# graphcore-research/bess-kge

Hardware: AMD Instinct MI355X
Metric: positive+negative triples scored/sec (higher is better)
Workload: dtype f32; 1 GPU; ogbl-biokg-shaped ComplEx d=256 fp32 (W=512), 93,773 entities per shard, n_shard=1, S=4096 positives x 256 per-triple negatives per GPU per step, EmbeddingMoving, mode=score (gather+score+loss); negatives_per_triple=256, mode=score, collectives=none

## Files before the change

bess-kge_amd/csrc/neg_pertriple.hip:

```cpp
#include "common.h"
#include "loss_rows.h"

namespace bess {

struct NegPtArgs {
    const float* query;
    const void* base;
    const int32_t* idx;
    int64_t n_query;
    int n_neg;
    int W;
    int nch;
    int nb;
    int items_per_query;
    float sign;
    int accum = 0;
    float p = 2.f;
    int dn_by_row = 0;
    int sweep_shift = -1;
};

struct FuseArgs {
    const float* pos;
    int kind;
    float beta;
    float margin;
    float shift;
    float* st_ml;
    float* st_acc;
    const uint8_t* mask = nullptr;
    int64_t mask_rows = 0;
    int mask_cols = 0, mask_from = 0;
};

__device__ __forceinline__ float sigmoid_f(float x) { return 1.f / (1.f + expf(-x)); }

template <typename T, int VEC, int IT, int RED, int UNROLL, bool FUSE>
__global__ __launch_bounds__(256) void k_neg_pertriple_fwd(NegPtArgs a, float* __restrict__ out,
                                                           int64_t ld_out, FuseArgs f) {
    const int lane = threadIdx.x & 63;
    const int g = lane & 15;
    const int sub = lane >> 4;
    const int64_t item = blockIdx.x * 4ll + (threadIdx.x >> 6);
    if (item >= a.n_query * a.items_per_query) return;
    const int64_t q = item / a.items_per_query;
    const int k0 = static_cast<int>(item - q * a.items_per_query) * a.nb;
    const int k1 = min(k0 + a.nb, a.n_neg);

    float qv[IT][VEC];
    const float* qp = a.query + q * a.W;
#pragma unroll
    for (int it = 0; it < IT; ++it) {
        load_chunk<float, VEC>(qp, g + 16 * it, a.nch, qv[it]);
    }

    const T* base = static_cast<const T*>(a.base);
    const int32_t* idx = a.idx + q * a.n_neg;
    float* orow = out + q * ld_out;
    float fm = -INFINITY, fl = 0.f, facc[IT][VEC];
    float fpos = 0.f;
    if (FUSE) {
#pragma unroll
        for (int it = 0; it < IT; ++it)
#pragma unroll
            for (int v = 0; v < VEC; ++v) facc[it][v] = 0.f;
        if (f.kind == BESS_LOSS_MARGIN) fpos = f.pos[q];
    }

    int32_t nrow[UNROLL];
#pragma unroll
    for (int u = 0; u < UNROLL; ++u) nrow[u] = idx[min(k0 + sub + 4 * u, k1 - 1)];
    for (int kb = k0; kb < k1; kb += 4 * UNROLL) {
        float ev[UNROLL][IT][VEC];
        bool valid[UNROLL];
#pragma unroll
        for (int u = 0; u < UNROLL; ++u) {
            const int k = kb + sub + 4 * u;
            valid[u] = k < k1;
            const T* rp = base + static_cast<int64_t>(nrow[u]) * a.W;
            nrow[u] = idx[min(k + 4 * UNROLL, k1 - 1)];
#pragma unroll
            for (int it = 0; it < IT; ++it) {
                load_chunk<T, VEC>(rp, g + 16 * it, a.nch, ev[u][it]);
            }
        }
#pragma unroll
        for (int u = 0; u < UNROLL; ++u) {
            float acc = 0.f;
#pragma unroll
            for (int it = 0; it < IT; ++it) {
#pragma unroll
                for (int v = 0; v < VEC; ++v) {
                    if (RED == RED_DOT) {
                        acc = fmaf(qv[it][v], ev[u][it][v], acc);
                    } else if (RED == RED_L1) {
                        acc += fabsf(qv[it][v] - ev[u][it][v]);
                    } else {
                        acc += lp_term(qv[it][v] - ev[u][it][v], a.p);
                    }
                }
            }
            acc = row16_allreduce_sum(acc);
            if (RED == RED_L2) acc = lp_root(acc, a.p);
            float sc = a.sign * acc;
            if (FUSE && f.mask && valid[u]) {
                const int kcol = kb + sub + 4 * u - f.mask_from;
                const int64_t mrow = f.mask_rows == 1 ? 0 : q;
                if (kcol >= 0 && f.mask[mrow * f.mask_cols + kcol] == 0) sc += BESS_BAD_NEGATIVE_SCORE;
            }
            if (g == 0 && valid[u]) orow[kb + sub + 4 * u] = a.accum ? orow[kb + sub + 4 * u] + sc : sc;
            if (FUSE && valid[u]) {
                const float z = f.beta * (sc + f.shift);
                const float m_new = fmaxf(fm, z);
                const float corr = expf(fm - m_new);
                const float e = expf(z - m_new);
                float gs = 1.f;
                if (f.kind == BESS_LOSS_LOGSIGMOID) gs = sigmoid_f(sc + f.margin);
                else if (f.kind == BESS_LOSS_MARGIN) gs = (sc - fpos + f.margin > 0.f) ? 1.f : 0.f;
                const float p = e * gs;
                fl = fmaf(fl, corr, e);
                fm = m_new;
                const float inv_norm = RED == RED_L2 ? lp_inv(acc, a.p) : 0.f;
#pragma unroll
                for (int it = 0; it < IT; ++it)
#pragma unroll
                    for (int v = 0; v < VEC; ++v) {
                        float dsdq;
                        if (RED == RED_DOT) dsdq = ev[u][it][v];
                        else if (RED == RED_L1) dsdq = -sgnf(qv[it][v] - ev[u][it][v]);
                        else dsdq = -lp_dterm(qv[it][v] - ev[u][it][v], a.p) * inv_norm;
                        facc[it][v] = fmaf(facc[it][v], corr, p * dsdq);
                    }
            }
        }
    }
    if (FUSE) {
        float m_all = fmaxf(fm, __shfl_xor(fm, 16, 64));
        m_all = fmaxf(m_all, __shfl_xor(m_all, 32, 64));
        const float sc = (fm == -INFINITY) ? 0.f : expf(fm - m_all);
        float l = fl * sc;
        l += __shfl_xor(l, 16, 64);
        l += __shfl_xor(l, 32, 64);
        const int64_t slot = q * a.items_per_query + (item - q * a.items_per_query);
        if (lane == 0) {
            f.st_ml[slot * 2 + 0] = m_all;
            f.st_ml[slot * 2 + 1] = l;
        }
        float* ap = f.st_acc + slot * a.W;
#pragma unroll
        for (int it = 0; it < IT; ++it) {
            const int c = g + 16 * it;
#pragma unroll
            for (int v = 0; v < VEC; ++v) {
                float x = facc[it][v] * sc;
                x += __shfl_xor(x, 16, 64);
                x += __shfl_xor(x, 32, 64);
                if (sub == 0 && c < a.nch) ap[c * VEC + v] = x;
            }
        }
    }
}

constexpr int SW_NB = 1024;
constexpr int SW_PMAX = 8192;
constexpr int SW_PPT = SW_PMAX / 256;
constexpr int SW_SHARE = SW_PMAX / 8;
constexpr int SW_QFLOATS = 16384;
constexpr int64_t SW_REUSE_MIN = 4;

struct SweepArgs {
    int qb;
    int kc;
    int n_kchunks;
    int shift;
    int qstride;
};

template <typename T, int VEC, int IT, int RED, int UNROLL>
__global__ __launch_bounds__(256) void k_neg_pertriple_fwd_sweep(NegPtArgs a, SweepArgs s, float* __restrict__ out,
                                                                 int64_t ld_out) {
    extern __shared__ __attribute__((aligned(16))) float qs[];
    __shared__ int hist[SW_NB + 4];
    __shared__ int2 ent[SW_SHARE];
    __shared__ int rk[2][SW_PPT * 4];
    __shared__ int wsum[4];
    __shared__ int cut[4];

    const int tid = threadIdx.x;
    const int lane = tid & 63;
    const int wave = tid >> 6;
    const int label = blockIdx.x & 7;
    const int bc = blockIdx.x >> 3;
    const int qblk = bc / s.n_kchunks;
    const int kch = bc - qblk * s.n_kchunks;
    const int64_t q0 = static_cast<int64_t>(qblk) * s.qb;
    const int nqb = static_cast<int>(min(static_cast<int64_t>(s.qb), a.n_query - q0));
    const int kc0 = kch * s.kc;
    const int kcn = min(s.kc, a.n_neg - kc0);
    const int P = nqb * kcn;
    const int lo = static_cast<int>((static_cast<int64_t>(label) * P) >> 3);
    const int hi = static_cast<int>((static_cast<int64_t>(label + 1) * P) >> 3);

    for (int i = tid; i < nqb * IT * 16; i += 256) {
        const int qi = i / (IT * 16);
        const int c = i - qi * (IT * 16);
        float v[VEC];
        load_chunk<float, VEC>(a.query + (q0 + qi) * a.W, c, a.nch, v);
#pragma unroll
        for (int j = 0; j < VEC; ++j) qs[qi * s.qstride + c * VEC + j] = v[j];
    }
    for (int b = tid; b < SW_NB; b += 256) hist[b] = 0;
    if (tid < 2) cut[tid] = -1;
    int rr[SW_PPT];
#pragma unroll
    for (int j = 0; j < SW_PPT; ++j) {
        const int p = tid + 256 * j;
        rr[j] = 0;
        if (p < P) {
            const int qi = p / kcn;
            rr[j] = a.idx[(q0 + qi) * a.n_neg + kc0 + (p - qi * kcn)];
        }
    }
    __syncthreads();
#pragma unroll
    for (int j = 0; j < SW_PPT; ++j)
        if (tid + 256 * j < P) atomicAdd(&hist[min(static_cast<unsigned>(rr[j]) >> s.shift, SW_NB - 1u)], 1);
    __syncthreads();

    {
        int c[4], sum = 0;
#pragma unroll
        for (int i = 0; i < 4; ++i) {
            c[i] = hist[4 * tid + i];
            sum += c[i];
        }
        int incl = sum;
#pragma unroll
        for (int off = 1; off < 64; off <<= 1) {
            const int y = __shfl_up(incl, off, 64);
            if (lane >= off) incl += y;
        }
        if (lane == 63) wsum[wave] = incl;
        __syncthreads();
        int run = incl - sum;
        for (int w = 0; w < wave; ++w) run += wsum[w];
#pragma unroll
        for (int i = 0; i < 4; ++i) {
            const int b = 4 * tid + i;
            hist[b] = run;
            if (run < lo && lo < run + c[i]) cut[0] = b;
            if (run < hi && hi < run + c[i]) cut[1] = b;
            run += c[i];
        }
        if (tid == 255) hist[SW_NB] = run;
    }
    __syncthreads();

    const int cut0 = cut[0], cut1 = cut[1];
    const uint64_t lt = (1ull << lane) - 1ull;
#pragma unroll
    for (int j = 0; j < SW_PPT; ++j) {
        const bool live = tid + 256 * j < P;
        const unsigned b = min(static_cast<unsigned>(rr[j]) >> s.shift, SW_NB - 1u);
        const uint64_t m0 = __ballot(live && static_cast<int>(b) == cut0);
        const uint64_t m1 = __ballot(live && static_cast<int>(b) == cut1);
        if (lane == 0) {
            rk[0][j * 4 + wave] = __popcll(m0);
            rk[1][j * 4 + wave] = __popcll(m1);
        }
    }
    __syncthreads();
    if (wave == 0) {
#pragma unroll
        for (int h = 0; h < 2; ++h) {
            const int x0 = rk[h][2 * lane], x1 = rk[h][2 * lane + 1];
            int incl = x0 + x1;
#pragma unroll
            for (int off = 1; off < 64; off <<= 1) {
                const int y = __shfl_up(incl, off, 64);
                if (lane >= off) incl += y;
            }
            rk[h][2 * lane] = incl - x0 - x1;
            rk[h][2 * lane + 1] = incl - x1;
        }
    }
    __syncthreads();

    int slot[SW_PPT];
#pragma unroll
    for (int j = 0; j < SW_PPT; ++j) {
        const bool live = tid + 256 * j < P;
        const unsigned b = min(static_cast<unsigned>(rr[j]) >> s.shift, SW_NB - 1u);
        const bool in0 = live && static_cast<int>(b) == cut0;
        const bool in1 = live && static_cast<int>(b) == cut1 && !in0;
        const uint64_t m0 = __ballot(in0);
        const uint64_t m1 = __ballot(in1);
        const int b0 = live ? hist[b] : 0, b1 = live ? hist[b + 1] : 0;
        slot[j] = -1;
        if (live) {
            if (in0 || in1) {
                const int r = in0 ? rk[0][j * 4 + wave] + __popcll(m0 & lt) : rk[1][j * 4 + wave] + __popcll(m1 & lt);
                const int pos = b0 + r;
                if (pos >= lo && pos < hi) slot[j] = pos - lo;
            } else if (b0 >= lo && b1 <= hi) {
                slot[j] = -2;
            }
        }
    }
    __syncthreads();
#pragma unroll
    for (int j = 0; j < SW_PPT; ++j) {
        const int p = tid + 256 * j;
        if (slot[j] == -1) continue;
        const unsigned b = min(static_cast<unsigned>(rr[j]) >> s.shift, SW_NB - 1u);
        const int e = slot[j] >= 0 ? slot[j] : atomicAdd(&hist[b], 1) - lo;
        const int qi = p / kcn;
        ent[e] = make_int2(rr[j], (qi << 16) | (p - qi * kcn));
    }
    __syncthreads();

    const int n = hi - lo;
    const int g = lane & 15;
    const int sub = lane >> 4;
    const T* base = static_cast<const T*>(a.base);
    int2 nx[UNROLL];
#pragma unroll
    for (int u = 0; u < UNROLL; ++u) nx[u] = ent[max(0, min(wave * 4 * UNROLL + sub + 4 * u, n - 1))];
    for (int e0 = wave * 4 * UNROLL; e0 < n; e0 += 16 * UNROLL) {
        float ev[UNROLL][IT][VEC];
        int2 cur[UNROLL];
        bool valid[UNROLL];
#pragma unroll
        for (int u = 0; u < UNROLL; ++u) {
            const int e = e0 + sub + 4 * u;
            valid[u] = e < n;
            cur[u] = nx[u];
            const T* rp = base + static_cast<int64_t>(cur[u].x) * a.W;
            nx[u] = ent[min(e + 16 * UNROLL, n - 1)];
#pragma unroll
            for (int it = 0; it < IT; ++it) load_chunk<T, VEC>(rp, g + 16 * it, a.nch, ev[u][it]);
        }
#pragma unroll
        for (int u = 0; u < UNROLL; ++u) {
            const int qi = cur[u].y >> 16;
            const int kk = cur[u].y & 0xffff;
            const float* qp = qs + qi * s.qstride;
            float acc = 0.f;
#pragma unroll
            for (int it = 0; it < IT; ++it) {
                float qv[VEC];
                VecLoad<float, VEC>::load(qp + (g + 16 * it) * VEC, qv);
#pragma unroll
                for (int v = 0; v < VEC; ++v) {
                    if (RED == RED_DOT) {
                        acc = fmaf(qv[v], ev[u][it][v], acc);
                    } else if (RED == RED_L1) {
                        acc += fabsf(qv[v] - ev[u][it][v]);
                    } else {
                        acc += lp_term(qv[v] - ev[u][it][v], a.p);
                    }
                }
            }
            acc = row16_allreduce_sum(acc);
            if (RED == RED_L2) acc = lp_root(acc, a.p);
            if (g == 0 && valid[u]) out[(q0 + qi) * ld_out + kc0 + kk] = a.sign * acc;
        }
    }
}

__global__ __launch_bounds__(256) void k_combine_dq(const float* __restrict__ st_ml, const float* __restrict__ st_acc,
                                                    int64_t n_query, int items, int W, int kind, float loss_scale,
                                                    const float* __restrict__ pos, const float* __restrict__ weight,
                                                    int64_t weight_len, const float* __restrict__ norm,
                                                    float* __restrict__ d_query) {
    const int64_t q = blockIdx.x * 4ll + (threadIdx.x >> 6);
    if (q >= n_query) return;
    combine_dq_row(st_ml, st_acc, q, items, W, kind, loss_scale, pos, weight, weight_len, norm, d_query + q * W, nullptr);
}

template <typename T, int VEC, int IT, int RED, int UNROLL>
__global__ __launch_bounds__(256) void k_neg_pertriple_bwd(NegPtArgs a,
                                                           const float* __restrict__ d_out,
                                                           int64_t ld_dout,
                                                           float* __restrict__ d_query,
                                                           float* __restrict__ d_neg) {
    const int lane = threadIdx.x & 63;
    const int g = lane & 15;
    const int sub = lane >> 4;
    const int64_t item = blockIdx.x * 4ll + (threadIdx.x >> 6);
    if (item >= a.n_query * a.items_per_query) return;
    const int64_t q = item / a.items_per_query;
    const int k0 = static_cast<int>(item - q * a.items_per_query) * a.nb;
    const int k1 = min(k0 + a.nb, a.n_neg);

    float qv[IT][VEC], dq[IT][VEC];
    const float* qp = a.query + q * a.W;
#pragma unroll
    for (int it = 0; it < IT; ++it) {
#pragma unroll
        for (int v = 0; v < VEC; ++v) dq[it][v] = 0.f;
        load_chunk<float, VEC>(qp, g + 16 * it, a.nch, qv[it]);
    }
    const T* base = static_cast<const T*>(a.base);
    const int32_t* idx = a.idx + q * a.n_neg;
    const float* grow = d_out + q * ld_dout;

    int32_t nrow[UNROLL];
    float ngo[UNROLL];
#pragma unroll
    for (int u = 0; u < UNROLL; ++u) {
        const int kk = min(k0 + sub + 4 * u, k1 - 1);
        nrow[u] = idx[kk];
        ngo[u] = grow[kk];
    }
    const bool need_rows = !(RED == RED_DOT && d_query == nullptr);
    for (int kb = k0; kb < k1; kb += 4 * UNROLL) {
        float ev[UNROLL][IT][VEC], go[UNROLL];
        int ks[UNROLL];
        int32_t row_now[UNROLL];
        bool valid[UNROLL];
#pragma unroll
        for (int u = 0; u < UNROLL; ++u) {
            const int k = kb + sub + 4 * u;
            valid[u] = k < k1;
            ks[u] = min(k, k1 - 1);
            const T* rp = base + static_cast<int64_t>(nrow[u]) * a.W;
            row_now[u] = nrow[u];
            go[u] = valid[u] ? a.sign * ngo[u] : 0.f;
            const int kn = min(k + 4 * UNROLL, k1 - 1);
            nrow[u] = idx[kn];
            ngo[u] = grow[kn];
            if (need_rows) {
#pragma unroll
                for (int it = 0; it < IT; ++it) load_chunk<T, VEC>(rp, g + 16 * it, a.nch, ev[u][it]);
            } else {
#pragma unroll
                for (int it = 0; it < IT; ++it)
#pragma unroll
                    for (int v = 0; v < VEC; ++v) ev[u][it][v] = 0.f;
            }
        }
#pragma unroll
        for (int u = 0; u < UNROLL; ++u) {
            float gg = go[u];
            if (RED == RED_L2) {
                float ss = 0.f;
#pragma unroll
                for (int it = 0; it < IT; ++it)
#pragma unroll
                    for (int v = 0; v < VEC; ++v) {
                        ss += lp_term(qv[it][v] - ev[u][it][v], a.p);
                    }
                ss = row16_allreduce_sum(ss);
                gg *= lp_inv(lp_root(ss, a.p), a.p);
            }
            float* dn = d_neg + (a.dn_by_row ? static_cast<int64_t>(row_now[u]) : q * a.n_neg + ks[u]) * a.W;
#pragma unroll
            for (int it = 0; it < IT; ++it) {
                const int c = g + 16 * it;
                float de[VEC];
#pragma unroll
                for (int v = 0; v < VEC; ++v) {
                    float dqe;
                    if (RED == RED_DOT) {
                        dqe = gg * ev[u][it][v];
                        de[v] = gg * qv[it][v];
                    } else if (RED == RED_L1) {
                        dqe = gg * sgnf(qv[it][v] - ev[u][it][v]);
                        de[v] = -dqe;
                    } else {
                        dqe = gg * lp_dterm(qv[it][v] - ev[u][it][v], a.p);
                        de[v] = -dqe;
                    }
                    dq[it][v] += dqe;
                }
                if (d_neg && valid[u] && c < a.nch) {
                    if constexpr (VEC == 4) {
                        typedef float f4 __attribute__((ext_vector_type(4)));
#pragma unroll
                        for (int v = 0; v < VEC; v += 4) {
                            f4 o = {de[v], de[v + 1], de[v + 2], de[v + 3]};
                            __builtin_nontemporal_store(o, reinterpret_cast<f4*>(dn + c * VEC + v));
                        }
                    } else {
#pragma unroll
                        for (int v = 0; v < VEC; ++v) dn[c * VEC + v] = de[v];
                    }
                }
            }
        }
    }
    if (!d_query) return;
    float* dqp = d_query + q * a.W;
#pragma unroll
    for (int it = 0; it < IT; ++it) {
        const int c = g + 16 * it;
#pragma unroll
        for (int v = 0; v < VEC; ++v) {
            float x = dq[it][v];
            x += __shfl_xor(x, 16, 64);
            x += __shfl_xor(x, 32, 64);
            if (sub == 0 && c < a.nch) {
                if (a.items_per_query == 1) dqp[c * VEC + v] = x;
                else unsafeAtomicAdd(dqp + c * VEC + v, x);
            }
        }
    }
}

template <typename T, int VEC, int IT, int RED>
static void launch_fwd(const NegPtArgs& a, float* out, int64_t ld, const FuseArgs* fuse, hipStream_t st) {
    const int64_t items = a.n_query * a.items_per_query;
    constexpr int EPL = IT * VEC;
    constexpr int UNROLL = EPL <= 16 ? 4 : (EPL <= 32 ? 2 : 1);
    if (!fuse && a.sweep_shift >= 0) {
        SweepArgs s;
        s.qstride = IT * 16 * VEC;
        s.qb = SW_QFLOATS / s.qstride < 32 ? SW_QFLOATS / s.qstride : 32;
        s.kc = a.n_neg < SW_PMAX / s.qb ? a.n_neg : SW_PMAX / s.qb;
        s.n_kchunks = static_cast<int>(ceil_div(a.n_neg, s.kc));
        s.shift = a.sweep_shift;
        const int64_t blocks = ceil_div(a.n_query, s.qb) * s.n_kchunks * 8;
        const int lds = s.qb * s.qstride * static_cast<int>(sizeof(float));
        k_neg_pertriple_fwd_sweep<T, VEC, IT, RED, UNROLL>
            <<<static_cast<unsigned>(blocks), 256, lds, st>>>(a, s, out, ld);
    } else if (fuse) {
        constexpr int FU = EPL <= 16 ? 2 : 1;
        k_neg_pertriple_fwd<T, VEC, IT, RED, FU, true><<<ceil_div(items, 4), 256, 0, st>>>(a, out, ld, *fuse);
    } else {
        k_neg_pertriple_fwd<T, VEC, IT, RED, UNROLL, false><<<ceil_div(items, 4), 256, 0, st>>>(a, out, ld, FuseArgs{});
    }
}
template <typename T, int VEC, int IT, int RED>
static void launch_bwd(const NegPtArgs& a, const float* d_out, int64_t ld, float* dq, float* dn,
                       hipStream_t st) {
    const int64_t items = a.n_query * a.items_per_query;
    constexpr int EPL = IT * VEC;
    constexpr int BU = EPL <= 16 ? 2 : 1;
    k_neg_pertriple_bwd<T, VEC, IT, RED, BU><<<ceil_div(items, 4), 256, 0, st>>>(a, d_out, ld, dq, dn);
}

template <typename T, int VEC, int IT>
static void by_red(int red, bool fwd, const NegPtArgs& a, float* out, const float* d_out, int64_t ld,
                   float* dq, float* dn, const FuseArgs* fuse, hipStream_t st) {
    switch (red) {
        case RED_DOT:
            fwd ? launch_fwd<T, VEC, IT, RED_DOT>(a, out, ld, fuse, st)
                : launch_bwd<T, VEC, IT, RED_DOT>(a, d_out, ld, dq, dn, st);
            break;
        case RED_L1:
            fwd ? launch_fwd<T, VEC, IT, RED_L1>(a, out, ld, fuse, st)
                : launch_bwd<T, VEC, IT, RED_L1>(a, d_out, ld, dq, dn, st);
            break;
        default:
            fwd ? launch_fwd<T, VEC, IT, RED_L2>(a, out, ld, fuse, st)
                : launch_bwd<T, VEC, IT, RED_L2>(a, d_out, ld, dq, dn, st);
    }
}

template <typename T, int VEC>
static int by_it(int it, int red, bool fwd, const NegPtArgs& a, float* out, const float* d_out,
                 int64_t ld, float* dq, float* dn, const FuseArgs* fuse, hipStream_t st) {
    if (it <= 1) by_red<T, VEC, 1>(red, fwd, a, out, d_out, ld, dq, dn, fuse, st);
    else if (it <= 2) by_red<T, VEC, 2>(red, fwd, a, out, d_out, ld, dq, dn, fuse, st);
    else if (it <= 4) by_red<T, VEC, 4>(red, fwd, a, out, d_out, ld, dq, dn, fuse, st);
    else if (it <= 8) by_red<T, VEC, 8>(red, fwd, a, out, d_out, ld, dq, dn, fuse, st);
    else if (it <= 16) by_red<T, VEC, 16>(red, fwd, a, out, d_out, ld, dq, dn, fuse, st);
    else return fail(BESS_EUNSUPPORTED, "neg_score_pertriple: row of %d scalars too wide", a.W);
    return BESS_OK;
}

static int negatives_per_item(int64_t n_query, int64_t n_neg, int64_t row_bytes) {
    int nb = 64;
    while (nb < 256 && nb * row_bytes < 131072) nb <<= 1;
    while (nb > 8 && n_query * ceil_div(n_neg, nb) < 256 * 16 * 2) nb >>= 1;
    return nb;
}

static int vec_of(const bess_model_desc* d) {
    const int maxvec = d->dtype == BESS_F32 ? 4 : 8;
    if (d->width % maxvec == 0) return maxvec;
    return (d->dtype == BESS_F16 && d->width % 2 == 0) ? 2 : 1;
}

static int sweep_shift_for(const bess_model_desc* d, int64_t n_query, int64_t n_neg) {
    if (d->scorer > BESS_COMPLEX || d->width > 16 * 16 * vec_of(d)) return -1;
    const int64_t rows = d->reserved[1];
    if (rows <= 0 || n_query <= 0 || n_neg <= 0 || n_query * n_neg < SW_REUSE_MIN * rows) return -1;
    if (ceil_div(n_query, 8) * ceil_div(n_neg, 256) * 8 >= (1ll << 31)) return -1;
    int shift = 0;
    while (((rows - 1) >> shift) >= SW_NB) ++shift;
    return shift;
}

static int run(const bess_model_desc* d, bool fwd, const float* query, int64_t n_query,
               const void* neg_base, const int32_t* neg_idx, int64_t n_neg, float* out,
               const float* d_out, int64_t ld, float* dq, float* dn, void* stream,
               const FuseArgs* fuse = nullptr) {
    if (int e = check_desc(d)) return e;
    BESS_REQUIRE(n_query >= 0 && n_neg >= 0 && n_neg < (1ll << 31), "neg_score_pertriple: bad sizes");
    if (n_query == 0 || n_neg == 0) return BESS_OK;
    BESS_REQUIRE(query && neg_base && neg_idx, "neg_score_pertriple: NULL pointer");
    BESS_REQUIRE(ld >= n_neg, "neg_score_pertriple: leading dimension %lld < n_neg %lld", (long long)ld,
                 (long long)n_neg);
    if (d->scorer == BESS_BOXE)
        return boxe_negatives(d, fwd, false, query, n_query, neg_base, neg_idx, n_neg, out, d_out, ld, dq, dn,
                              as_stream(stream));
    if (d->scorer == BESS_AFFINE)
        return affine_pertriple(d, fwd, query, n_query, neg_base, neg_idx, n_neg, out, d_out, ld, dq, dn,
                                as_stream(stream));
    const int W = d->width;
    const int vec = vec_of(d);
    NegPtArgs a;
    a.query = query;
    a.base = neg_base;
    a.idx = neg_idx;
    a.n_query = n_query;
    a.n_neg = static_cast<int>(n_neg);
    a.W = W;
    a.nch = W / vec;
    a.nb = negatives_per_item(n_query, n_neg, static_cast<int64_t>(W) * (d->dtype == BESS_F32 ? 4 : 2));
    a.items_per_query = static_cast<int>(ceil_div(n_neg, a.nb));
    a.sign = is_distance(d->scorer) ? -1.f : 1.f;
    a.p = static_cast<float>(d->norm_p);
    a.dn_by_row = (!fwd && (d->reserved[0] & BESS_FLAG_DNEG_BY_ROW)) ? 1 : 0;
    if (fwd && !fuse) a.sweep_shift = sweep_shift_for(d, n_query, n_neg);
    const int red = reduce_of(d);
    hipStream_t st = as_stream(stream);
    if (!fwd && a.items_per_query > 1 && dq) {
        hipError_t e = fill_words_async(dq, 0u, n_query * W, st);
        if (e != hipSuccess) return fail(static_cast<int>(e), "memset d_query: %s", hipGetErrorString(e));
    }
    const int max_cols = 16 * 16 * vec;
    if (W > max_cols) {
        if (red == RED_L2)
            return fail(BESS_EUNSUPPORTED, "neg_score_pertriple: p = 2 on rows of %d scalars (more than %d)", W, max_cols);
        if (fuse)
            return fail(BESS_EUNSUPPORTED, "neg_score_pertriple: fused training forward on rows of %d scalars (more than %d)",
                        W, max_cols);
    }
    const int64_t sz = d->dtype == BESS_F32 ? 4 : 2;
    for (int col0 = 0; col0 < W; col0 += max_cols) {
        const int cols = W - col0 < max_cols ? W - col0 : max_cols;
        NegPtArgs w = a;
        w.query = query + col0;
        w.base = static_cast<const char*>(neg_base) + col0 * sz;
        w.nch = cols / vec;
        w.accum = col0 > 0;
        const int it = static_cast<int>(ceil_div(w.nch, 16));
        float* dqw = dq ? dq + col0 : nullptr;
        float* dnw = dn ? dn + col0 : nullptr;
        int rc = BESS_OK;
        if (d->dtype == BESS_F32) {
            if (vec == 4) rc = by_it<float, 4>(it, red, fwd, w, out, d_out, ld, dqw, dnw, fuse, st);
            else rc = by_it<float, 1>(it, red, fwd, w, out, d_out, ld, dqw, dnw, fuse, st);
        } else {
            if (vec == 8) rc = by_it<half_t, 8>(it, red, fwd, w, out, d_out, ld, dqw, dnw, fuse, st);
            else if (vec == 2) rc = by_it<half_t, 2>(it, red, fwd, w, out, d_out, ld, dqw, dnw, fuse, st);
            else rc = by_it<half_t, 1>(it, red, fwd, w, out, d_out, ld, dqw, dnw, fuse, st);
        }
        if (rc) return rc;
    }
    return check_launch(fwd ? "neg_score_pertriple_fwd" : "neg_score_pertriple_bwd");
}

}

extern "C" int bess_neg_score_pertriple_fwd(const bess_model_desc* d, const float* query,
                                            int64_t n_query, const void* neg_base,
                                            const int32_t* neg_idx, int64_t n_neg, float* out,
                                            int64_t ld_out, void* stream) {
    if (n_query > 0 && n_neg > 0 && !out) return bess::fail(BESS_EINVAL, "neg_score_pertriple_fwd: NULL out");
    return bess::run(d, true, query, n_query, neg_base, neg_idx, n_neg, out, nullptr, ld_out, nullptr,
                     nullptr, stream);
}

extern "C" int bess_neg_score_pertriple_bwd(const bess_model_desc* d, const float* query,
                                            int64_t n_query, const void* neg_base,
                                            const int32_t* neg_idx, int64_t n_neg,
                                            const float* d_out, int64_t ld_dout, float* d_query,
                                            float* d_neg, void* stream) {
    if (n_query > 0 && n_neg > 0 && !(d_out && (d_query || d_neg)))
        return bess::fail(BESS_EINVAL, "neg_score_pertriple_bwd: NULL pointer");
    return bess::run(d, false, query, n_query, neg_base, neg_idx, n_neg, nullptr, d_out, ld_dout,
                     d_query, d_neg, stream);
}

extern "C" int bess_neg_pertriple_sweep(const bess_model_desc* d, int64_t n_query, int64_t n_neg, int32_t* sweep) {
    if (int e = bess::check_desc(d)) return e;
    if (!sweep || n_query < 0 || n_neg < 0) return bess::fail(BESS_EINVAL, "neg_pertriple_sweep: bad argument");
    *sweep = bess::sweep_shift_for(d, n_query, n_neg) >= 0 ? 1 : 0;
    return BESS_OK;
}

static int64_t row_bytes_of(const bess_model_desc* d) {
    return static_cast<int64_t>(d->width) * (d->dtype == BESS_F32 ? 4 : 2);
}

extern "C" int bess_neg_pertriple_items(const bess_model_desc* d, int64_t n_query, int64_t n_neg, int32_t* items) {
    if (!d || !items || n_query < 0 || n_neg < 0) return bess::fail(BESS_EINVAL, "neg_pertriple_items: bad argument");
    *items = n_neg > 0 ? static_cast<int32_t>(bess::ceil_div(n_neg, bess::negatives_per_item(n_query, n_neg, row_bytes_of(d))))
                       : 0;
    return BESS_OK;
}

extern "C" int bess_neg_score_pertriple_fwd_dq(const bess_model_desc* d, const bess_loss_desc* l, const float* query,
                                               int64_t n_query, const void* neg_base, const int32_t* neg_idx,
                                               int64_t n_neg, const float* pos, const float* weight,
                                               int64_t weight_len, float* out, int64_t ld_out, float* d_query,
                                               float* state_ml, float* state_acc, void* stream) {
    return bess_neg_score_pertriple_fwd_dq_masked(d, l, query, n_query, neg_base, neg_idx, n_neg, pos, weight, weight_len,
                                                  nullptr, 0, 0, out, ld_out, d_query, state_ml, state_acc, stream);
}

extern "C" int bess_neg_score_pertriple_fwd_dq_masked(const bess_model_desc* d, const bess_loss_desc* l,
                                                      const float* query, int64_t n_query, const void* neg_base,
                                                      const int32_t* neg_idx, int64_t n_neg, const float* pos,
                                                      const float* weight, int64_t weight_len, const uint8_t* mask,
                                                      int64_t mask_rows, int64_t mask_cols, float* out,
                                                      int64_t ld_out, float* d_query, float* state_ml,
                                                      float* state_acc, void* stream) {
    using namespace bess;
    if (int e = check_desc(d)) return e;
    BESS_REQUIRE(l, "neg_score_pertriple_fwd_dq: NULL loss descriptor");
    BESS_REQUIRE(d->scorer <= BESS_COMPLEX, "neg_score_pertriple_fwd_dq: scorer %d has no fused form", d->scorer);
    BESS_REQUIRE(l->kind == BESS_LOSS_LOGSIGMOID || l->kind == BESS_LOSS_MARGIN || l->kind == BESS_LOSS_SSCE,
                 "neg_score_pertriple_fwd_dq: unknown loss %d", l->kind);
    if (n_query <= 0 || n_neg <= 0) return BESS_OK;
    BESS_REQUIRE(out && state_ml && state_acc && weight && (weight_len == 1 || weight_len == n_query),
                 "neg_score_pertriple_fwd_dq: NULL pointer or bad weight length");
    BESS_REQUIRE(pos || l->kind == BESS_LOSS_LOGSIGMOID, "neg_score_pertriple_fwd_dq: this loss needs the positive scores");
    FuseArgs f;
    f.pos = pos;
    f.kind = l->kind;
    f.beta = l->kind == BESS_LOSS_SSCE ? 1.f : (l->adversarial ? l->adversarial_scale : 0.f);
    f.margin = l->margin;
    f.shift = l->kind == BESS_LOSS_SSCE ? l->ssce_shift : 0.f;
    f.st_ml = state_ml;
    f.st_acc = state_acc;
    if (mask) {
        BESS_REQUIRE(mask_cols > 0 && mask_cols <= n_neg && (mask_rows == 1 || mask_rows == n_query),
                     "neg_score_pertriple_fwd_dq_masked: mask [%lld, %lld] for %lld queries x %lld negatives",
                     (long long)mask_rows, (long long)mask_cols, (long long)n_query, (long long)n_neg);
        f.mask = mask;
        f.mask_rows = mask_rows;
        f.mask_cols = static_cast<int>(mask_cols);
        f.mask_from = static_cast<int>(n_neg - mask_cols);
    }
    const int rc = run(d, true, query, n_query, neg_base, neg_idx, n_neg, out, nullptr, ld_out, nullptr, nullptr, stream,
                       &f);
    if (rc) return rc;
    const int items = static_cast<int>(ceil_div(n_neg, negatives_per_item(n_query, n_neg, row_bytes_of(d))));
    if (!d_query) return BESS_OK;
    k_combine_dq<<<static_cast<unsigned>(ceil_div(n_query, 4)), 256, 0, as_stream(stream)>>>(
        state_ml, state_acc, n_query, items, d->width, l->kind, l->loss_scale, pos, weight, weight_len, nullptr, d_query);
    return check_launch("neg_score_pertriple_fwd_dq");
}

extern "C" int bess_neg_score_pertriple_fwd_partials(const bess_model_desc* d, const bess_loss_desc* l,
                                                     const float* query, int64_t n_query, const void* neg_base,
                                                     const int32_t* neg_idx, int64_t n_neg, float* out,
                                                     int64_t ld_out, float* state_ml, float* state_acc, void* stream) {
    using namespace bess;
    if (int e = check_desc(d)) return e;
    BESS_REQUIRE(l, "neg_score_pertriple_fwd_partials: NULL loss descriptor");
    BESS_REQUIRE(d->scorer <= BESS_COMPLEX, "neg_score_pertriple_fwd_partials: scorer %d has no fused form", d->scorer);
    if (l->kind != BESS_LOSS_LOGSIGMOID && l->kind != BESS_LOSS_SSCE)
        return fail(BESS_EUNSUPPORTED, "neg_score_pertriple_fwd_partials: loss %d weighs a negative by the positive score, "
                                       "which the scoring shard does not have", l->kind);
    if (n_query <= 0 || n_neg <= 0) return BESS_OK;
    BESS_REQUIRE(out && state_ml && state_acc, "neg_score_pertriple_fwd_partials: NULL pointer");
    FuseArgs f;
    f.pos = nullptr;
    f.kind = l->kind;
    f.beta = l->kind == BESS_LOSS_SSCE ? 1.f : (l->adversarial ? l->adversarial_scale : 0.f);
    f.margin = l->margin;
    f.shift = l->kind == BESS_LOSS_SSCE ? l->ssce_shift : 0.f;
    f.st_ml = state_ml;
    f.st_acc = state_acc;
    return run(d, true, query, n_query, neg_base, neg_idx, n_neg, out, nullptr, ld_out, nullptr, nullptr, stream, &f);
}

extern "C" int bess_combine_dq_partials(const float* state_ml, const float* state_acc, int64_t n_query, int32_t items,
                                        int32_t width, const float* norm, float* d_query, void* stream) {
    using namespace bess;
    BESS_REQUIRE(n_query >= 0 && items > 0 && width > 0, "combine_dq_partials: bad sizes");
    if (n_query == 0) return BESS_OK;
    BESS_REQUIRE(state_ml && state_acc && norm && d_query, "combine_dq_partials: NULL pointer");
    k_combine_dq<<<static_cast<unsigned>(ceil_div(n_query, 4)), 256, 0, as_stream(stream)>>>(
        state_ml, state_acc, n_query, items, width, 0, 1.f, nullptr, nullptr, 1, norm, d_query);
    return check_launch("combine_dq_partials");
}
```

Baseline: 5.159 billion triples/s.

## Widen sweep kernel to 512 threads and batch query staging loads

Templates the sweep forward kernel on workgroup size and query-block cap, and defaults it to 512 threads instead of 256, so each thread holds half as many pair indices and eight waves share one staged query block. Query staging into shared memory now issues a batch of loads before the stores, and the index loads are moved ahead of the histogram clear. Per-pair bucket indices are kept in registers instead of being recomputed. Larger workgroups may lower occupancy and raise register pressure. Env-var tuning hooks are compiled in only under BESS_SW_TUNE.

```diff
diff --git a/bess-kge_amd/csrc/neg_pertriple.hip b/bess-kge_amd/csrc/neg_pertriple.hip
--- a/bess-kge_amd/csrc/neg_pertriple.hip
+++ b/bess-kge_amd/csrc/neg_pertriple.hip
@@ -1,5 +1,9 @@
 #include "common.h"
 #include "loss_rows.h"
+#ifdef BESS_SW_TUNE
+#include <cstdlib>
+#include <cstring>
+#endif
 
 namespace bess {
 
@@ -163,27 +167,42 @@
 
 constexpr int SW_NB = 1024;
 constexpr int SW_PMAX = 8192;
-constexpr int SW_PPT = SW_PMAX / 256;
 constexpr int SW_SHARE = SW_PMAX / 8;
 constexpr int SW_QFLOATS = 16384;
+constexpr int SW_THREADS = 512;
+constexpr int SW_QBMAX = 32;
+constexpr int SW_STAGE_BATCH = 8;
 constexpr int64_t SW_REUSE_MIN = 4;
 
+constexpr int sweep_qb(int qbmax, int qstride) { return SW_QFLOATS / qstride < qbmax ? SW_QFLOATS / qstride : qbmax; }
+
 struct SweepArgs {
-    int qb;
     int kc;
     int n_kchunks;
     int shift;
-    int qstride;
+#ifdef BESS_SW_TUNE
+    int mode = 0;
+#endif
 };
 
-template <typename T, int VEC, int IT, int RED, int UNROLL>
-__global__ __launch_bounds__(256) void k_neg_pertriple_fwd_sweep(NegPtArgs a, SweepArgs s, float* __restrict__ out,
-                                                                 int64_t ld_out) {
+template <typename T, int VEC, int IT, int RED, int UNROLL, int THREADS, int QBMAX>
+__global__ __launch_bounds__(THREADS) void k_neg_pertriple_fwd_sweep(NegPtArgs a, SweepArgs s, float* __restrict__ out,
+                                                                     int64_t ld_out) {
+    constexpr int NW = THREADS / 64;
+    constexpr int PPT = SW_PMAX / THREADS;
+    constexpr int BPT = SW_NB / THREADS;
+    constexpr int NRK = PPT * NW;
+    constexpr int QSTRIDE = IT * 16 * VEC;
+    constexpr int QB = sweep_qb(QBMAX, QSTRIDE);
+    static_assert(THREADS % 64 == 0 && SW_PMAX % THREADS == 0 && SW_NB % THREADS == 0 && BPT >= 1, "workgroup shape");
+    static_assert(NRK == 2 * 64, "wave 0 scans two rank cells per lane");
+    static_assert(QB >= 1 && QB * QSTRIDE <= SW_QFLOATS, "staged queries");
+    static_assert(QB <= 32 && SW_PMAX < (1 << 16), "ent packing: qi << 16 | k - kc0, k - kc0 < kc <= SW_PMAX");
     extern __shared__ __attribute__((aligned(16))) float qs[];
     __shared__ int hist[SW_NB + 4];
     __shared__ int2 ent[SW_SHARE];
-    __shared__ int rk[2][SW_PPT * 4];
-    __shared__ int wsum[4];
+    __shared__ int rk[2][NRK];
+    __shared__ int wsum[(NW + 3) / 4 * 4];
     __shared__ int cut[4];
 
     const int tid = threadIdx.x;
@@ -193,45 +212,84 @@
     const int bc = blockIdx.x >> 3;
     const int qblk = bc / s.n_kchunks;
     const int kch = bc - qblk * s.n_kchunks;
-    const int64_t q0 = static_cast<int64_t>(qblk) * s.qb;
-    const int nqb = static_cast<int>(min(static_cast<int64_t>(s.qb), a.n_query - q0));
+    const int64_t q0 = static_cast<int64_t>(qblk) * QB;
+    const int nqb = static_cast<int>(min(static_cast<int64_t>(QB), a.n_query - q0));
     const int kc0 = kch * s.kc;
     const int kcn = min(s.kc, a.n_neg - kc0);
     const int P = nqb * kcn;
     const int lo = static_cast<int>((static_cast<int64_t>(label) * P) >> 3);
     const int hi = static_cast<int>((static_cast<int64_t>(label + 1) * P) >> 3);
 
-    for (int i = tid; i < nqb * IT * 16; i += 256) {
-        const int qi = i / (IT * 16);
-        const int c = i - qi * (IT * 16);
-        float v[VEC];
-        load_chunk<float, VEC>(a.query + (q0 + qi) * a.W, c, a.nch, v);
-#pragma unroll
-        for (int j = 0; j < VEC; ++j) qs[qi * s.qstride + c * VEC + j] = v[j];
-    }
-    for (int b = tid; b < SW_NB; b += 256) hist[b] = 0;
-    if (tid < 2) cut[tid] = -1;
-    int rr[SW_PPT];
-#pragma unroll
-    for (int j = 0; j < SW_PPT; ++j) {
-        const int p = tid + 256 * j;
+    int rr[PPT];
+#pragma unroll
+    for (int j = 0; j < PPT; ++j) {
+        const int p = tid + THREADS * j;
         rr[j] = 0;
         if (p < P) {
             const int qi = p / kcn;
             rr[j] = a.idx[(q0 + qi) * a.n_neg + kc0 + (p - qi * kcn)];
         }
     }
+    for (int b = tid; b < SW_NB; b += THREADS) hist[b] = 0;
+    if (tid < 2) cut[tid] = -1;
+    constexpr int QCHUNKS = QB * IT * 16;
+    if (nqb == QB) {
+#pragma unroll
+        for (int i0 = 0; i0 < QCHUNKS; i0 += THREADS * SW_STAGE_BATCH) {
+            float v[SW_STAGE_BATCH][VEC];
+#pragma unroll
+            for (int u = 0; u < SW_STAGE_BATCH; ++u) {
+                if (i0 + THREADS * u < QCHUNKS) {
+                    const int i = min(i0 + THREADS * u + tid, QCHUNKS - 1);
+                    const int qi = i / (IT * 16);
+                    load_chunk<float, VEC>(a.query + (q0 + qi) * a.W, i - qi * (IT * 16), a.nch, v[u]);
+                }
+            }
+#pragma unroll
+            for (int u = 0; u < SW_STAGE_BATCH; ++u) {
+                const int i = i0 + THREADS * u + tid;
+                if (i0 + THREADS * u < QCHUNKS && i < QCHUNKS) {
+#pragma unroll
+                    for (int j = 0; j < VEC; ++j) qs[i * VEC + j] = v[u][j];
+                }
+            }
+        }
+    } else {
+        for (int i = tid; i < nqb * IT * 16; i += THREADS) {
+            const int qi = i / (IT * 16);
+            float v[VEC];
+            load_chunk<float, VEC>(a.query + (q0 + qi) * a.W, i - qi * (IT * 16), a.nch, v);
+#pragma unroll
+            for (int j = 0; j < VEC; ++j) qs[i * VEC + j] = v[j];
+        }
+    }
     __syncthreads();
-#pragma unroll
-    for (int j = 0; j < SW_PPT; ++j)
-        if (tid + 256 * j < P) atomicAdd(&hist[min(static_cast<unsigned>(rr[j]) >> s.shift, SW_NB - 1u)], 1);
+#ifdef BESS_SW_TUNE
+    if (s.mode == 2) {
+#pragma unroll
+        for (int j = 0; j < PPT; ++j) {
+            const int p = tid + THREADS * j;
+            if (p >= lo && p < hi) {
+                const int qi = p / kcn;
+                ent[p - lo] = make_int2(rr[j], (qi << 16) | (p - qi * kcn));
+            }
+        }
+        __syncthreads();
+    } else {
+#endif
+    int bk[PPT];
+#pragma unroll
+    for (int j = 0; j < PPT; ++j) bk[j] = static_cast<int>(min(static_cast<unsigned>(rr[j]) >> s.shift, SW_NB - 1u));
+#pragma unroll
+    for (int j = 0; j < PPT; ++j)
+        if (tid + THREADS * j < P) atomicAdd(&hist[bk[j]], 1);
     __syncthreads();
 
     {
-        int c[4], sum = 0;
-#pragma unroll
-        for (int i = 0; i < 4; ++i) {
-            c[i] = hist[4 * tid + i];
+        int c[BPT], sum = 0;
+#pragma unroll
+        for (int i = 0; i < BPT; ++i) {
+            c[i] = hist[BPT * tid + i];
             sum += c[i];
         }
         int incl = sum;
@@ -245,28 +303,27 @@
         int run = incl - sum;
         for (int w = 0; w < wave; ++w) run += wsum[w];
 #pragma unroll
-        for (int i = 0; i < 4; ++i) {
-            const int b = 4 * tid + i;
+        for (int i = 0; i < BPT; ++i) {
+            const int b = BPT * tid + i;
             hist[b] = run;
             if (run < lo && lo < run + c[i]) cut[0] = b;
             if (run < hi && hi < run + c[i]) cut[1] = b;
             run += c[i];
         }
-        if (tid == 255) hist[SW_NB] = run;
+        if (tid == THREADS - 1) hist[SW_NB] = run;
     }
     __syncthreads();
 
     const int cut0 = cut[0], cut1 = cut[1];
     const uint64_t lt = (1ull << lane) - 1ull;
 #pragma unroll
-    for (int j = 0; j < SW_PPT; ++j) {
-        const bool live = tid + 256 * j < P;
-        const unsigned b = min(static_cast<unsigned>(rr[j]) >> s.shift, SW_NB - 1u);
-        const uint64_t m0 = __ballot(live && static_cast<int>(b) == cut0);
-        const uint64_t m1 = __ballot(live && static_cast<int>(b) == cut1);
+    for (int j = 0; j < PPT; ++j) {
+        const bool live = tid + THREADS * j < P;
+        const uint64_t m0 = __ballot(live && bk[j] == cut0);
+        const uint64_t m1 = __ballot(live && bk[j] == cut1);
         if (lane == 0) {
-            rk[0][j * 4 + wave] = __popcll(m0);
-            rk[1][j * 4 + wave] = __popcll(m1);
+            rk[0][j * NW + wave] = __popcll(m0);
+            rk[1][j * NW + wave] = __popcll(m1);
         }
     }
     __syncthreads();
@@ -286,20 +343,19 @@
     }
     __syncthreads();
 
-    int slot[SW_PPT];
-#pragma unroll
-    for (int j = 0; j < SW_PPT; ++j) {
-        const bool live = tid + 256 * j < P;
-        const unsigned b = min(static_cast<unsigned>(rr[j]) >> s.shift, SW_NB - 1u);
-        const bool in0 = live && static_cast<int>(b) == cut0;
-        const bool in1 = live && static_cast<int>(b) == cut1 && !in0;
+    int slot[PPT];
+#pragma unroll
+    for (int j = 0; j < PPT; ++j) {
+        const bool live = tid + THREADS * j < P;
+        const bool in0 = live && bk[j] == cut0;
+        const bool in1 = live && bk[j] == cut1 && !in0;
         const uint64_t m0 = __ballot(in0);
         const uint64_t m1 = __ballot(in1);
-        const int b0 = live ? hist[b] : 0, b1 = live ? hist[b + 1] : 0;
+        const int b0 = live ? hist[bk[j]] : 0, b1 = live ? hist[bk[j] + 1] : 0;
         slot[j] = -1;
         if (live) {
             if (in0 || in1) {
-                const int r = in0 ? rk[0][j * 4 + wave] + __popcll(m0 & lt) : rk[1][j * 4 + wave] + __popcll(m1 & lt);
+                const int r = in0 ? rk[0][j * NW + wave] + __popcll(m0 & lt) : rk[1][j * NW + wave] + __popcll(m1 & lt);
                 const int pos = b0 + r;
                 if (pos >= lo && pos < hi) slot[j] = pos - lo;
             } else if (b0 >= lo && b1 <= hi) {
@@ -309,15 +365,21 @@
     }
     __syncthreads();
 #pragma unroll
-    for (int j = 0; j < SW_PPT; ++j) {
-        const int p = tid + 256 * j;
+    for (int j = 0; j < PPT; ++j) {
+        const int p = tid + THREADS * j;
         if (slot[j] == -1) continue;
-        const unsigned b = min(static_cast<unsigned>(rr[j]) >> s.shift, SW_NB - 1u);
-        const int e = slot[j] >= 0 ? slot[j] : atomicAdd(&hist[b], 1) - lo;
+        const int e = slot[j] >= 0 ? slot[j] : atomicAdd(&hist[bk[j]], 1) - lo;
         const int qi = p / kcn;
         ent[e] = make_int2(rr[j], (qi << 16) | (p - qi * kcn));
     }
     __syncthreads();
+#ifdef BESS_SW_TUNE
+    }
+    if (s.mode == 1) {
+        if (tid == 0 && label == 0 && hi > lo) out[q0 * ld_out + kc0] = static_cast<float>(ent[0].x + ent[hi - lo - 1].y);
+        return;
+    }
+#endif
 
     const int n = hi - lo;
     const int g = lane & 15;
@@ -326,7 +388,7 @@
     int2 nx[UNROLL];
 #pragma unroll
     for (int u = 0; u < UNROLL; ++u) nx[u] = ent[max(0, min(wave * 4 * UNROLL + sub + 4 * u, n - 1))];
-    for (int e0 = wave * 4 * UNROLL; e0 < n; e0 += 16 * UNROLL) {
+    for (int e0 = wave * 4 * UNROLL; e0 < n; e0 += NW * 4 * UNROLL) {
         float ev[UNROLL][IT][VEC];
         int2 cur[UNROLL];
         bool valid[UNROLL];
@@ -336,7 +398,7 @@
             valid[u] = e < n;
             cur[u] = nx[u];
             const T* rp = base + static_cast<int64_t>(cur[u].x) * a.W;
-            nx[u] = ent[min(e + 16 * UNROLL, n - 1)];
+            nx[u] = ent[min(e + NW * 4 * UNROLL, n - 1)];
 #pragma unroll
             for (int it = 0; it < IT; ++it) load_chunk<T, VEC>(rp, g + 16 * it, a.nch, ev[u][it]);
         }
@@ -344,7 +406,7 @@
         for (int u = 0; u < UNROLL; ++u) {
             const int qi = cur[u].y >> 16;
             const int kk = cur[u].y & 0xffff;
-            const float* qp = qs + qi * s.qstride;
+            const float* qp = qs + qi * QSTRIDE;
             float acc = 0.f;
 #pragma unroll
             for (int it = 0; it < IT; ++it) {
@@ -508,22 +570,49 @@
     }
 }
 
+struct SweepGeom {
+    int qb, kc, n_kchunks;
+    int64_t blocks;
+    int lds;
+};
+static SweepGeom sweep_geom(int64_t n_query, int n_neg, int qbmax, int qstride) {
+    SweepGeom g;
+    g.qb = sweep_qb(qbmax, qstride);
+    g.kc = n_neg < SW_PMAX / g.qb ? n_neg : SW_PMAX / g.qb;
+    g.n_kchunks = static_cast<int>(ceil_div(n_neg, g.kc));
+    g.blocks = ceil_div(n_query, g.qb) * g.n_kchunks * 8;
+    g.lds = g.qb * qstride * static_cast<int>(sizeof(float));
+    return g;
+}
+template <typename T, int VEC, int IT, int RED, int UNROLL, int THREADS, int QBMAX>
+static void launch_sweep(const NegPtArgs& a, float* out, int64_t ld, hipStream_t st) {
+    const SweepGeom g = sweep_geom(a.n_query, a.n_neg, QBMAX, IT * 16 * VEC);
+    SweepArgs s;
+    s.kc = g.kc;
+    s.n_kchunks = g.n_kchunks;
+    s.shift = a.sweep_shift;
+#ifdef BESS_SW_TUNE
+    const char* m = getenv("BESS_SW_MODE");
+    s.mode = m ? atoi(m) : 0;
+#endif
+    k_neg_pertriple_fwd_sweep<T, VEC, IT, RED, UNROLL, THREADS, QBMAX>
+        <<<static_cast<unsigned>(g.blocks), THREADS, g.lds, st>>>(a, s, out, ld);
+}
 template <typename T, int VEC, int IT, int RED>
 static void launch_fwd(const NegPtArgs& a, float* out, int64_t ld, const FuseArgs* fuse, hipStream_t st) {
     const int64_t items = a.n_query * a.items_per_query;
     constexpr int EPL = IT * VEC;
     constexpr int UNROLL = EPL <= 16 ? 4 : (EPL <= 32 ? 2 : 1);
     if (!fuse && a.sweep_shift >= 0) {
-        SweepArgs s;
-        s.qstride = IT * 16 * VEC;
-        s.qb = SW_QFLOATS / s.qstride < 32 ? SW_QFLOATS / s.qstride : 32;
-        s.kc = a.n_neg < SW_PMAX / s.qb ? a.n_neg : SW_PMAX / s.qb;
-        s.n_kchunks = static_cast<int>(ceil_div(a.n_neg, s.kc));
-        s.shift = a.sweep_shift;
-        const int64_t blocks = ceil_div(a.n_query, s.qb) * s.n_kchunks * 8;
-        const int lds = s.qb * s.qstride * static_cast<int>(sizeof(float));
-        k_neg_pertriple_fwd_sweep<T, VEC, IT, RED, UNROLL>
-            <<<static_cast<unsigned>(blocks), 256, lds, st>>>(a, s, out, ld);
+#ifdef BESS_SW_TUNE
+        const char* ev = getenv("BESS_SW_SHAPE");
+        const int shape = ev ? atoi(ev) * 100 + atoi(strchr(ev, 'x') ? strchr(ev, 'x') + 1 : "32") : SW_THREADS * 100 + SW_QBMAX;
+        if (shape == 25632) launch_sweep<T, VEC, IT, RED, UNROLL, 256, 32>(a, out, ld, st);
+        else if (shape == 25616) launch_sweep<T, VEC, IT, RED, UNROLL, 256, 16>(a, out, ld, st);
+        else if (shape == 51216) launch_sweep<T, VEC, IT, RED, UNROLL, 512, 16>(a, out, ld, st);
+        else
+#endif
+        launch_sweep<T, VEC, IT, RED, UNROLL, SW_THREADS, SW_QBMAX>(a, out, ld, st);
     } else if (fuse) {
         constexpr int FU = EPL <= 16 ? 2 : 1;
         k_neg_pertriple_fwd<T, VEC, IT, RED, FU, true><<<ceil_div(items, 4), 256, 0, st>>>(a, out, ld, *fuse);
```

Measured after the change: 5.031 billion triples/s. -2.5%, worse.

## Widen sweep kernel blocks, double-buffer row gathers, overlap query staging, alternate sweep order

Applied to the files above, without the earlier changes.

Templates the sort-and-sweep forward kernel on thread count and uses 512 threads when IT is small. The query tile is loaded into registers alongside the index loads and written to LDS after bucketing, so its global latency overlaps the histogram work. The gather loop gains an A/B double buffer that issues the next embedding-row loads before scoring the current ones. Every other wave of resident blocks walks its entries in reverse, using an occupancy-derived residency count, to improve cache reuse across consecutive blocks. These add register pressure and occupancy queries, and idle waves now exit early.

```diff
diff --git a/bess-kge_amd/csrc/neg_pertriple.hip b/bess-kge_amd/csrc/neg_pertriple.hip
--- a/bess-kge_amd/csrc/neg_pertriple.hip
+++ b/bess-kge_amd/csrc/neg_pertriple.hip
@@ -1,3 +1,5 @@
+#include <limits.h>
+
 #include "common.h"
 #include "loss_rows.h"
 
@@ -163,7 +165,6 @@
 
 constexpr int SW_NB = 1024;
 constexpr int SW_PMAX = 8192;
-constexpr int SW_PPT = SW_PMAX / 256;
 constexpr int SW_SHARE = SW_PMAX / 8;
 constexpr int SW_QFLOATS = 16384;
 constexpr int64_t SW_REUSE_MIN = 4;
@@ -174,16 +175,24 @@
     int n_kchunks;
     int shift;
     int qstride;
+    int resident;
 };
 
-template <typename T, int VEC, int IT, int RED, int UNROLL>
-__global__ __launch_bounds__(256) void k_neg_pertriple_fwd_sweep(NegPtArgs a, SweepArgs s, float* __restrict__ out,
-                                                                 int64_t ld_out) {
+template <typename T, int VEC, int IT, int RED, int UNROLL, int NT>
+__global__ __launch_bounds__(NT, NT / 128) void k_neg_pertriple_fwd_sweep(NegPtArgs a, SweepArgs s, float* __restrict__ out,
+                                                                int64_t ld_out) {
+    constexpr int NW = NT / 64;
+    constexpr int PPT = SW_PMAX / NT;
+    constexpr int BPT = SW_NB / NT;
+    constexpr int NRK = PPT * NW;
+    constexpr int QB = SW_QFLOATS / (IT * 16 * VEC) < 32 ? SW_QFLOATS / (IT * 16 * VEC) : 32;
+    constexpr int QPT = (QB * IT * 16 + NT - 1) / NT;
+    static_assert(NRK == 128 && BPT >= 1, "rank scan: two cells per lane of wave 0");
     extern __shared__ __attribute__((aligned(16))) float qs[];
     __shared__ int hist[SW_NB + 4];
     __shared__ int2 ent[SW_SHARE];
-    __shared__ int rk[2][SW_PPT * 4];
-    __shared__ int wsum[4];
+    __shared__ int rk[2][NRK];
+    __shared__ int wsum[8];
     __shared__ int cut[4];
 
     const int tid = threadIdx.x;
@@ -201,37 +210,36 @@
     const int lo = static_cast<int>((static_cast<int64_t>(label) * P) >> 3);
     const int hi = static_cast<int>((static_cast<int64_t>(label + 1) * P) >> 3);
 
-    for (int i = tid; i < nqb * IT * 16; i += 256) {
-        const int qi = i / (IT * 16);
-        const int c = i - qi * (IT * 16);
-        float v[VEC];
-        load_chunk<float, VEC>(a.query + (q0 + qi) * a.W, c, a.nch, v);
-#pragma unroll
-        for (int j = 0; j < VEC; ++j) qs[qi * s.qstride + c * VEC + j] = v[j];
-    }
-    for (int b = tid; b < SW_NB; b += 256) hist[b] = 0;
+    for (int b = tid; b < SW_NB; b += NT) hist[b] = 0;
     if (tid < 2) cut[tid] = -1;
-    int rr[SW_PPT];
-#pragma unroll
-    for (int j = 0; j < SW_PPT; ++j) {
-        const int p = tid + 256 * j;
+    int rr[PPT];
+#pragma unroll
+    for (int j = 0; j < PPT; ++j) {
+        const int p = tid + NT * j;
         rr[j] = 0;
         if (p < P) {
             const int qi = p / kcn;
             rr[j] = a.idx[(q0 + qi) * a.n_neg + kc0 + (p - qi * kcn)];
         }
     }
+    float qreg[QPT][VEC];
+#pragma unroll
+    for (int k = 0; k < QPT; ++k) {
+        const int i = min(tid + NT * k, nqb * IT * 16 - 1);
+        const int qi = i / (IT * 16);
+        load_chunk<float, VEC>(a.query + (q0 + qi) * a.W, i - qi * (IT * 16), a.nch, qreg[k]);
+    }
     __syncthreads();
 #pragma unroll
-    for (int j = 0; j < SW_PPT; ++j)
-        if (tid + 256 * j < P) atomicAdd(&hist[min(static_cast<unsigned>(rr[j]) >> s.shift, SW_NB - 1u)], 1);
+    for (int j = 0; j < PPT; ++j)
+        if (tid + NT * j < P) atomicAdd(&hist[min(static_cast<unsigned>(rr[j]) >> s.shift, SW_NB - 1u)], 1);
     __syncthreads();
 
     {
-        int c[4], sum = 0;
-#pragma unroll
-        for (int i = 0; i < 4; ++i) {
-            c[i] = hist[4 * tid + i];
+        int c[BPT], sum = 0;
+#pragma unroll
+        for (int i = 0; i < BPT; ++i) {
+            c[i] = hist[BPT * tid + i];
             sum += c[i];
         }
         int incl = sum;
@@ -245,28 +253,28 @@
         int run = incl - sum;
         for (int w = 0; w < wave; ++w) run += wsum[w];
 #pragma unroll
-        for (int i = 0; i < 4; ++i) {
-            const int b = 4 * tid + i;
+        for (int i = 0; i < BPT; ++i) {
+            const int b = BPT * tid + i;
             hist[b] = run;
             if (run < lo && lo < run + c[i]) cut[0] = b;
             if (run < hi && hi < run + c[i]) cut[1] = b;
             run += c[i];
         }
-        if (tid == 255) hist[SW_NB] = run;
+        if (tid == NT - 1) hist[SW_NB] = run;
     }
     __syncthreads();
 
     const int cut0 = cut[0], cut1 = cut[1];
     const uint64_t lt = (1ull << lane) - 1ull;
 #pragma unroll
-    for (int j = 0; j < SW_PPT; ++j) {
-        const bool live = tid + 256 * j < P;
+    for (int j = 0; j < PPT; ++j) {
+        const bool live = tid + NT * j < P;
         const unsigned b = min(static_cast<unsigned>(rr[j]) >> s.shift, SW_NB - 1u);
         const uint64_t m0 = __ballot(live && static_cast<int>(b) == cut0);
         const uint64_t m1 = __ballot(live && static_cast<int>(b) == cut1);
         if (lane == 0) {
-            rk[0][j * 4 + wave] = __popcll(m0);
-            rk[1][j * 4 + wave] = __popcll(m1);
+            rk[0][j * NW + wave] = __popcll(m0);
+            rk[1][j * NW + wave] = __popcll(m1);
         }
     }
     __syncthreads();
@@ -286,10 +294,10 @@
     }
     __syncthreads();
 
-    int slot[SW_PPT];
-#pragma unroll
-    for (int j = 0; j < SW_PPT; ++j) {
-        const bool live = tid + 256 * j < P;
+    int slot[PPT];
+#pragma unroll
+    for (int j = 0; j < PPT; ++j) {
+        const bool live = tid + NT * j < P;
         const unsigned b = min(static_cast<unsigned>(rr[j]) >> s.shift, SW_NB - 1u);
         const bool in0 = live && static_cast<int>(b) == cut0;
         const bool in1 = live && static_cast<int>(b) == cut1 && !in0;
@@ -299,7 +307,7 @@
         slot[j] = -1;
         if (live) {
             if (in0 || in1) {
-                const int r = in0 ? rk[0][j * 4 + wave] + __popcll(m0 & lt) : rk[1][j * 4 + wave] + __popcll(m1 & lt);
+                const int r = in0 ? rk[0][j * NW + wave] + __popcll(m0 & lt) : rk[1][j * NW + wave] + __popcll(m1 & lt);
                 const int pos = b0 + r;
                 if (pos >= lo && pos < hi) slot[j] = pos - lo;
             } else if (b0 >= lo && b1 <= hi) {
@@ -309,61 +317,120 @@
     }
     __syncthreads();
 #pragma unroll
-    for (int j = 0; j < SW_PPT; ++j) {
-        const int p = tid + 256 * j;
+    for (int j = 0; j < PPT; ++j) {
+        const int p = tid + NT * j;
         if (slot[j] == -1) continue;
         const unsigned b = min(static_cast<unsigned>(rr[j]) >> s.shift, SW_NB - 1u);
         const int e = slot[j] >= 0 ? slot[j] : atomicAdd(&hist[b], 1) - lo;
         const int qi = p / kcn;
         ent[e] = make_int2(rr[j], (qi << 16) | (p - qi * kcn));
     }
+#pragma unroll
+    for (int k = 0; k < QPT; ++k) {
+        const int i = tid + NT * k;
+        if (i < nqb * IT * 16) {
+            const int qi = i / (IT * 16);
+            float* dst = qs + qi * s.qstride + (i - qi * (IT * 16)) * VEC;
+#pragma unroll
+            for (int j = 0; j < VEC; ++j) dst[j] = qreg[k][j];
+        }
+    }
     __syncthreads();
 
     const int n = hi - lo;
+    if (wave * 4 * UNROLL >= n) return;
     const int g = lane & 15;
     const int sub = lane >> 4;
     const T* base = static_cast<const T*>(a.base);
-    int2 nx[UNROLL];
-#pragma unroll
-    for (int u = 0; u < UNROLL; ++u) nx[u] = ent[max(0, min(wave * 4 * UNROLL + sub + 4 * u, n - 1))];
-    for (int e0 = wave * 4 * UNROLL; e0 < n; e0 += 16 * UNROLL) {
-        float ev[UNROLL][IT][VEC];
-        int2 cur[UNROLL];
-        bool valid[UNROLL];
-#pragma unroll
-        for (int u = 0; u < UNROLL; ++u) {
-            const int e = e0 + sub + 4 * u;
-            valid[u] = e < n;
-            cur[u] = nx[u];
-            const T* rp = base + static_cast<int64_t>(cur[u].x) * a.W;
-            nx[u] = ent[min(e + 16 * UNROLL, n - 1)];
-#pragma unroll
-            for (int it = 0; it < IT; ++it) load_chunk<T, VEC>(rp, g + 16 * it, a.nch, ev[u][it]);
-        }
-#pragma unroll
-        for (int u = 0; u < UNROLL; ++u) {
-            const int qi = cur[u].y >> 16;
-            const int kk = cur[u].y & 0xffff;
-            const float* qp = qs + qi * s.qstride;
-            float acc = 0.f;
-#pragma unroll
-            for (int it = 0; it < IT; ++it) {
-                float qv[VEC];
-                VecLoad<float, VEC>::load(qp + (g + 16 * it) * VEC, qv);
-#pragma unroll
-                for (int v = 0; v < VEC; ++v) {
-                    if (RED == RED_DOT) {
-                        acc = fmaf(qv[v], ev[u][it][v], acc);
-                    } else if (RED == RED_L1) {
-                        acc += fabsf(qv[v] - ev[u][it][v]);
-                    } else {
-                        acc += lp_term(qv[v] - ev[u][it][v], a.p);
-                    }
+    const bool rev = ((blockIdx.x / static_cast<unsigned>(s.resident)) & 1u) != 0;
+    auto entry = [&](int e) {
+        e = min(e, n - 1);
+        return ent[rev ? n - 1 - e : e];
+    };
+    auto score = [&](int e, int2 c, const float (&ev)[IT][VEC]) {
+        const int qi = c.y >> 16;
+        const int kk = c.y & 0xffff;
+        const float* qp = qs + qi * s.qstride;
+        float acc = 0.f;
+#pragma unroll
+        for (int it = 0; it < IT; ++it) {
+            float qv[VEC];
+            VecLoad<float, VEC>::load(qp + (g + 16 * it) * VEC, qv);
+            const bool live = g + 16 * it < a.nch;
+#pragma unroll
+            for (int v = 0; v < VEC; ++v) {
+                const float x = live ? ev[it][v] : 0.f;
+                if (RED == RED_DOT) {
+                    acc = fmaf(qv[v], x, acc);
+                } else if (RED == RED_L1) {
+                    acc += fabsf(qv[v] - x);
+                } else {
+                    acc += lp_term(qv[v] - x, a.p);
                 }
             }
-            acc = row16_allreduce_sum(acc);
-            if (RED == RED_L2) acc = lp_root(acc, a.p);
-            if (g == 0 && valid[u]) out[(q0 + qi) * ld_out + kc0 + kk] = a.sign * acc;
+        }
+        acc = row16_allreduce_sum(acc);
+        if (RED == RED_L2) acc = lp_root(acc, a.p);
+        if (g == 0 && e < n) out[(q0 + qi) * ld_out + kc0 + kk] = a.sign * acc;
+    };
+    constexpr int STEP = 4 * UNROLL * NW;
+    if constexpr (UNROLL >= 2) {
+        constexpr int U = UNROLL / 2;
+        float evA[U][IT][VEC], evB[U][IT][VEC];
+        int2 curA[U], curB[U], nx[U];
+        int e0 = wave * 4 * UNROLL;
+#pragma unroll
+        for (int u = 0; u < U; ++u) {
+            curA[u] = entry(e0 + sub + 4 * u);
+            curB[u] = entry(e0 + sub + 4 * (u + U));
+        }
+#pragma unroll
+        for (int u = 0; u < U; ++u) {
+            const T* rp = base + static_cast<int64_t>(curA[u].x) * a.W;
+#pragma unroll
+            for (int it = 0; it < IT; ++it) load_chunk_clamped<T, VEC>(rp, g + 16 * it, a.nch, evA[u][it]);
+        }
+        for (; e0 < n; e0 += STEP) {
+#pragma unroll
+            for (int u = 0; u < U; ++u) {
+                const T* rp = base + static_cast<int64_t>(curB[u].x) * a.W;
+#pragma unroll
+                for (int it = 0; it < IT; ++it) load_chunk_clamped<T, VEC>(rp, g + 16 * it, a.nch, evB[u][it]);
+                nx[u] = entry(e0 + STEP + sub + 4 * u);
+            }
+#pragma unroll
+            for (int u = 0; u < U; ++u) score(e0 + sub + 4 * u, curA[u], evA[u]);
+#pragma unroll
+            for (int u = 0; u < U; ++u) {
+                curA[u] = nx[u];
+                const T* rp = base + static_cast<int64_t>(curA[u].x) * a.W;
+#pragma unroll
+                for (int it = 0; it < IT; ++it) load_chunk_clamped<T, VEC>(rp, g + 16 * it, a.nch, evA[u][it]);
+                nx[u] = entry(e0 + STEP + sub + 4 * (u + U));
+            }
+#pragma unroll
+            for (int u = 0; u < U; ++u) {
+                score(e0 + sub + 4 * (u + U), curB[u], evB[u]);
+                curB[u] = nx[u];
+            }
+        }
+    } else {
+        int2 nx[UNROLL];
+#pragma unroll
+        for (int u = 0; u < UNROLL; ++u) nx[u] = entry(wave * 4 * UNROLL + sub + 4 * u);
+        for (int e0 = wave * 4 * UNROLL; e0 < n; e0 += STEP) {
+            float ev[UNROLL][IT][VEC];
+            int2 cur[UNROLL];
+#pragma unroll
+            for (int u = 0; u < UNROLL; ++u) {
+                cur[u] = nx[u];
+                const T* rp = base + static_cast<int64_t>(cur[u].x) * a.W;
+                nx[u] = entry(e0 + STEP + sub + 4 * u);
+#pragma unroll
+                for (int it = 0; it < IT; ++it) load_chunk_clamped<T, VEC>(rp, g + 16 * it, a.nch, ev[u][it]);
+            }
+#pragma unroll
+            for (int u = 0; u < UNROLL; ++u) score(e0 + sub + 4 * u, cur[u], ev[u]);
         }
     }
 }
@@ -522,8 +589,18 @@
         s.shift = a.sweep_shift;
         const int64_t blocks = ceil_div(a.n_query, s.qb) * s.n_kchunks * 8;
         const int lds = s.qb * s.qstride * static_cast<int>(sizeof(float));
-        k_neg_pertriple_fwd_sweep<T, VEC, IT, RED, UNROLL>
-            <<<static_cast<unsigned>(blocks), 256, lds, st>>>(a, s, out, ld);
+        constexpr int NT = IT <= 8 ? 512 : 256;
+        const auto kern = k_neg_pertriple_fwd_sweep<T, VEC, IT, RED, UNROLL, NT>;
+        static const int resident = [&] {
+            int dev = 0, cus = 0, per_cu = 0;
+            if (hipGetDevice(&dev) != hipSuccess ||
+                hipDeviceGetAttribute(&cus, hipDeviceAttributeMultiprocessorCount, dev) != hipSuccess ||
+                hipOccupancyMaxActiveBlocksPerMultiprocessor(&per_cu, kern, NT, lds) != hipSuccess || per_cu * cus <= 0)
+                return INT_MAX;
+            return per_cu * cus;
+        }();
+        s.resident = resident;
+        kern<<<static_cast<unsigned>(blocks), NT, lds, st>>>(a, s, out, ld);
     } else if (fuse) {
         constexpr int FU = EPL <= 16 ? 2 : 1;
         k_neg_pertriple_fwd<T, VEC, IT, RED, FU, true><<<ceil_div(items, 4), 256, 0, st>>>(a, out, ld, *fuse);
```

Result: slower. 5.160 billion triples/s before, 4.725 billion triples/s after (-8.4%).
